# talha-alam/ADAM-Dehaze

Hardware: AMD Instinct MI355X
Metric: images/sec CORUN-Complex fwd+bwd 512x1024 bs=8; PSNR vs CPU ref (higher is better)
Workload: dtype f32; 1 GPU; CORUN-Complex (HighIntensityDehazeModel base 96) train-mode fwd + L1 + bwd + Adam; per_gpu_batch=8, global_batch=8, height=512, width=1024, parallelism=dp1

## Files before the change

adam-dehaze_amd/csrc/bn_act.hip:

```cpp
#include "common.h"

__global__ __launch_bounds__(1024) void bn_finalize_kernel(const float* __restrict__ partials, int nblk, int NcP, int C,
                                                           double count, const float* __restrict__ gamma,
                                                           const float* __restrict__ beta, float eps, float momentum,
                                                           float* running_mean, float* running_var, float* scale,
                                                           float* shift, float* save_mean, float* save_invstd, int64_t* num_batches_tracked) {
    __shared__ double red[2][32][33];
    int c;
    double S, Q, mean, var;
    if (!bn_column_sums<4>(partials, nblk, NcP, C, red, c, S, Q)) return;
    bn_mean_var(S, Q, count, mean, var);
    bn_fold_channel(c, mean, var, count, gamma, beta, eps, momentum, running_mean, running_var, scale, shift, save_mean,
                    save_invstd, num_batches_tracked);
}

extern "C" int adh_bn_finalize(void* stream, const float* partials, int nblk, int NcP, int C, double count,
                               const float* gamma, const float* beta, float eps, float momentum, float* running_mean,
                               float* running_var, float* scale, float* shift, float* save_mean, float* save_invstd,
                               int64_t* num_batches_tracked) {
    if (!partials || !scale || !shift || nblk < 1 || C < 1 || NcP < C || count <= 0) return ADH_E_ARG;
    hipLaunchKernelGGL(bn_finalize_kernel, dim3(adh_ceil_div(C, 32)), dim3(1024), 0, (hipStream_t)stream, partials, nblk,
                       NcP, C, count, gamma, beta, eps, momentum, running_mean, running_var, scale, shift, save_mean,
                       save_invstd, num_batches_tracked);
    return adh_check_launch();
}

__global__ __launch_bounds__(1024) void bn_partial_sums_kernel(const float* __restrict__ partials, int nblk, int pitch, int C,
                                                               double count, double* __restrict__ sums) {
    __shared__ double red[2][32][33];
    int c;
    double S, Q;
    if (bn_column_sums<2>(partials, nblk, pitch, C, red, c, S, Q)) {
        sums[c] = S;
        sums[C + c] = Q;
    }
    if (blockIdx.x == 0 && threadIdx.x == 0) sums[2 * C] = count;
}

extern "C" int adh_bn_partial_sums(void* stream, const float* partials, int nblk, int pitch, int C, double count, double* sums) {
    if (!partials || !sums || nblk < 1 || C < 1 || pitch < C || count <= 0) return ADH_E_ARG;
    hipLaunchKernelGGL(bn_partial_sums_kernel, dim3(adh_ceil_div(C, 32)), dim3(1024), 0, (hipStream_t)stream, partials, nblk,
                       pitch, C, count, sums);
    return adh_check_launch();
}

__global__ void bn_finalize_sums_kernel(const double* __restrict__ sums, int C, const float* __restrict__ gamma,
                                        const float* __restrict__ beta, float eps, float momentum, float* running_mean,
                                        float* running_var, float* scale, float* shift, float* save_mean, float* save_invstd,
                                        int64_t* num_batches_tracked) {
    const int c = blockIdx.x * blockDim.x + threadIdx.x;
    if (c >= C) return;
    const double count = sums[2 * C];
    double mean, var;
    bn_mean_var(sums[c], sums[C + c], count, mean, var);
    bn_fold_channel(c, mean, var, count, gamma, beta, eps, momentum, running_mean, running_var, scale, shift, save_mean,
                    save_invstd, num_batches_tracked);
}

extern "C" int adh_bn_finalize_sums(void* stream, const double* sums, int C, const float* gamma, const float* beta, float eps,
                                    float momentum, float* running_mean, float* running_var, float* scale, float* shift,
                                    float* save_mean, float* save_invstd, int64_t* num_batches_tracked) {
    if (!sums || !scale || !shift || C < 1) return ADH_E_ARG;
    hipLaunchKernelGGL(bn_finalize_sums_kernel, dim3(adh_ceil_div(C, 128)), dim3(128), 0, (hipStream_t)stream, sums, C, gamma,
                       beta, eps, momentum, running_mean, running_var, scale, shift, save_mean, save_invstd, num_batches_tracked);
    return adh_check_launch();
}

__global__ void bn_bwd_finalize_sums_kernel(const double* __restrict__ local_sums, const double* __restrict__ global_sums, int C,
                                            const float* gamma, const float* invstd, float* dgamma, float* dbeta,
                                            int accumulate, float* coef) {
    const int c = blockIdx.x * blockDim.x + threadIdx.x;
    if (c >= C) return;
    const double count = global_sums[2 * C];
    bn_bwd_coef_channel(c, C, local_sums[c], local_sums[C + c], global_sums[c], global_sums[C + c], count, gamma, invstd, dgamma,
// ... 124 lines not shown
        const f32x4 mu = *reinterpret_cast<const f32x4*>(mean + c);
        const f32x4 is = *reinterpret_cast<const f32x4*>(invstd + c);
        f32x4 msc = {0.f, 0.f, 0.f, 0.f}, msh = msc;
        if (mask_ss) {
            msc = *reinterpret_cast<const f32x4*>(mask_ss + c);
            msh = *reinterpret_cast<const f32x4*>(mask_ss + C + c);
        }
        const int64_t p0 = (int64_t)blockIdx.x * BNB_PPB;
        const int64_t p1 = p0 + BNB_PPB < P ? p0 + BNB_PPB : P;
        for (int64_t p = p0 + prow; p < p1; p += BNB_UNROLL * R) {
            f32x4 g[BNB_UNROLL], o[BNB_UNROLL], yy[BNB_UNROLL];
            int mb[BNB_UNROLL];
#pragma unroll
            for (int u = 0; u < BNB_UNROLL; ++u) {
                const int64_t q = p + u * R < p1 ? p + u * R : p;
                g[u] = __builtin_nontemporal_load(reinterpret_cast<const f32x4*>(g_out + q * g_cs + c));
                if (mask_bits) mb[u] = mask_bits[(q * (C / 4) + (c >> 2)) >> 1] >> (4 * ((c >> 2) & 1));
                else if (act == ADH_ACT_RELU && !mask_ss) o[u] = __builtin_nontemporal_load(reinterpret_cast<const f32x4*>(out + q * out_cs + c));
                yy[u] = __builtin_nontemporal_load(reinterpret_cast<const f32x4*>(y + q * y_cs + c));
            }
#pragma unroll
            for (int u = 0; u < BNB_UNROLL; ++u) {
                if (p + u * R < p1) {
                    const f32x4 gg = bn_masked_grad(g[u], act, mask_bits != nullptr, mb[u], mask_ss != nullptr, yy[u], msc, msh, o[u]);
                    sg += gg;
                    sgx += gg * ((yy[u] - mu) * is);
                }
            }
        }
    }
    bn_block_fold(red, sg, sgx, CQ, R, c, C, partials);
  }
}

extern "C" int adh_bn_bwd_reduce(void* stream, const float* g_out, int g_cs, const float* out, int out_cs, int act,
                                 const float* y, int y_cs, const float* mean, const float* invstd, float* partials,
                                 int64_t P, int C, const float* mask_ss, const uint8_t* mask_bits) {
    if (!g_out || !y || !mean || !invstd || !partials || P < 1 || C < 4 || (C & 3) || C > 4096) return ADH_E_ARG;
    if (act == ADH_ACT_RELU && !out && !mask_ss && !mask_bits) return ADH_E_ARG;
    if (mask_bits && (((C / 4) & 1) || act != ADH_ACT_RELU)) return ADH_E_ARG;
    if (!adh_act_host_valid(act) || (act > ADH_ACT_RELU && !mask_ss)) return ADH_E_ARG;
    hipLaunchKernelGGL(bn_bwd_reduce_kernel, dim3(adh_bn_bwd_num_blocks(P, C)), dim3(256), 0, (hipStream_t)stream, g_out,
                       g_cs, out, out_cs, act, y, y_cs, mean, invstd, partials, P, C, mask_ss, mask_bits);
    return adh_check_launch();
}

__global__ __launch_bounds__(1024) void bn_bwd_finalize_kernel(const float* __restrict__ partials, int nblk, int pitch, int C,
                                                               double count, const float* gamma, const float* invstd,
                                                               float* dgamma, float* dbeta, int accumulate, float* coef,
                                                               int centered) {
    __shared__ double red[2][32][33];
    int c;
    double S, Q;
    if (!bn_column_sums<4>(partials, nblk, pitch, C, red, c, S, Q)) return;
    if (centered) Q *= (double)invstd[c];
    bn_bwd_coef_channel(c, C, S, Q, S, Q, count, gamma, invstd, dgamma, dbeta, accumulate, coef);
}

extern "C" int adh_bn_bwd_finalize(void* stream, const float* partials, int nblk, int C, double count,
                                   const float* gamma, const float* invstd, float* dgamma, float* dbeta, int accumulate,
                                   float* coef) {
    if (!partials || !invstd || !coef || nblk < 1 || C < 1 || count <= 0) return ADH_E_ARG;
    hipLaunchKernelGGL(bn_bwd_finalize_kernel, dim3(adh_ceil_div(C, 32)), dim3(1024), 0, (hipStream_t)stream, partials,
                       nblk, C, C, count, gamma, invstd, dgamma, dbeta, accumulate, coef, 0);
    return adh_check_launch();
}

extern "C" int adh_bn_bwd_finalize_centered(void* stream, const float* partials, int nblk, int pitch, int C, double count,
                                            const float* gamma, const float* invstd, float* dgamma, float* dbeta,
                                            int accumulate, float* coef) {
    if (!partials || !invstd || !coef || nblk < 1 || C < 1 || pitch < C || count <= 0) return ADH_E_ARG;
    hipLaunchKernelGGL(bn_bwd_finalize_kernel, dim3(adh_ceil_div(C, 32)), dim3(1024), 0, (hipStream_t)stream, partials,
                       nblk, pitch, C, count, gamma, invstd, dgamma, dbeta, accumulate, coef, 1);
    return adh_check_launch();
}

__global__ __launch_bounds__(256) void bn_bwd_apply_kernel(const float* __restrict__ g_out, int g_cs,
                                                           const float* __restrict__ out, int out_cs, int act,
                                                           const float* __restrict__ y, int y_cs,
                                                           const float* __restrict__ mean,
                                                           const float* __restrict__ invstd,
                                                           const float* __restrict__ coef, int training,
                                                           float* __restrict__ g_y, int gy_cs, float* __restrict__ g_res,
                                                           int gres_cs, int64_t P, int C, const float* __restrict__ mask_ss,
                                                           const uint8_t* __restrict__ mask_bits) {
    const int CQ = C / 4;
    int64_t p, pstep;
    int c;
    adh_stream_decode(CQ, p, pstep, c);
    const f32x4 k0 = *reinterpret_cast<const f32x4*>(coef + c);
    f32x4 mg = {0.f, 0.f, 0.f, 0.f}, kx = mg, mu = mg, msc = mg, msh = mg;
    if (mask_ss) {
        msc = *reinterpret_cast<const f32x4*>(mask_ss + c);
        msh = *reinterpret_cast<const f32x4*>(mask_ss + C + c);
    }
    if (training) {
        mg = *reinterpret_cast<const f32x4*>(coef + C + c);
        const f32x4 mgx = *reinterpret_cast<const f32x4*>(coef + 2 * C + c);
        mu = *reinterpret_cast<const f32x4*>(mean + c);
        kx = *reinterpret_cast<const f32x4*>(invstd + c) * mgx;
    }
    for (; p < P; p += EW_UNROLL * pstep) {
        f32x4 g[EW_UNROLL], o[EW_UNROLL], yy[EW_UNROLL];
        int mb[EW_UNROLL];
#pragma unroll
        for (int u = 0; u < EW_UNROLL; ++u) {
            const int64_t q = p + u * pstep < P ? p + u * pstep : p;
            g[u] = __builtin_nontemporal_load(reinterpret_cast<const f32x4*>(g_out + q * g_cs + c));
            if (mask_bits) mb[u] = mask_bits[(q * CQ + (c >> 2)) >> 1] >> (4 * ((c >> 2) & 1));
            else if (act == ADH_ACT_RELU && !mask_ss) o[u] = __builtin_nontemporal_load(reinterpret_cast<const f32x4*>(out + q * out_cs + c));
            if (training || mask_ss) yy[u] = __builtin_nontemporal_load(reinterpret_cast<const f32x4*>(y + q * y_cs + c));
        }
#pragma unroll
        for (int u = 0; u < EW_UNROLL; ++u) {
            const int64_t q = p + u * pstep;
            if (q < P) {
                f32x4 gg = g[u];
                if (mask_bits) {
#pragma unroll
                    for (int j = 0; j < 4; ++j) gg[j] = ((mb[u] >> j) & 1) ? gg[j] : 0.f;
                } else if (act == ADH_ACT_RELU) {
#pragma unroll
                    for (int j = 0; j < 4; ++j) {
                        const float ov = mask_ss ? fmaf(yy[u][j], msc[j], msh[j]) : o[u][j];
                        gg[j] = ov > 0.f ? gg[j] : 0.f;
// ... 31 lines not shown
```

adam-dehaze_amd/csrc/bn_stream.h:

```cpp
#pragma once

__host__ __device__ static inline bool adh_act_valid(int act) {
    return act == ADH_ACT_NONE || act == ADH_ACT_RELU || act == ADH_ACT_RELU6 || act == ADH_ACT_HARDSWISH ||
           act == ADH_ACT_HARDSIGMOID;
}
static inline bool adh_act_host_valid(int act) { return adh_act_valid(act); }
__device__ __forceinline__ float adh_act_fwd(int act, float z) {
    switch (act) {
        case ADH_ACT_RELU: return fmaxf(z, 0.f);
        case ADH_ACT_RELU6: return fminf(fmaxf(z, 0.f), 6.f);
        case ADH_ACT_HARDSWISH: return z * fminf(fmaxf(z + 3.f, 0.f), 6.f) / 6.f;
        case ADH_ACT_HARDSIGMOID: return fminf(fmaxf(z + 3.f, 0.f), 6.f) / 6.f;
        default: return z;
    }
}
__device__ __forceinline__ float adh_act_bwd(int act, float z, float g) {
    switch (act) {
        case ADH_ACT_RELU: return z > 0.f ? g : 0.f;
        case ADH_ACT_RELU6: return (z > 0.f && z < 6.f) ? g : 0.f;
        case ADH_ACT_HARDSWISH: return z <= -3.f ? 0.f : (z < 3.f ? g * (z / 3.f + 0.5f) : g);
        case ADH_ACT_HARDSIGMOID: return (z > -3.f && z < 3.f) ? g / 6.f : 0.f;
        default: return g;
    }
}
// ... 7 lines not shown
    int64_t blocks = (want + mult - 1) / mult * mult;
    if (blocks < mult) blocks = mult;
    return (int)blocks;
}
__device__ __forceinline__ void adh_stream_decode(int CQ, int64_t& p, int64_t& pstep, int& c) {
    const int64_t t = blockIdx.x * (int64_t)256 + threadIdx.x;
    pstep = (int64_t)gridDim.x * 256 / CQ;
    p = t / CQ;
    c = (int)(t - p * CQ) * 4;
}

__device__ __forceinline__ f32x4 bn_masked_grad(f32x4 gg, int act, bool bits, const int& mb, bool ss, const f32x4& yy,
                                                const f32x4& msc, const f32x4& msh, const f32x4& o) {
    if (bits) {
#pragma unroll
        for (int j = 0; j < 4; ++j) gg[j] = ((mb >> j) & 1) ? gg[j] : 0.f;
    } else if (act == ADH_ACT_RELU) {
#pragma unroll
        for (int j = 0; j < 4; ++j) {
            const float ov = ss ? fmaf(yy[j], msc[j], msh[j]) : o[j];
            gg[j] = ov > 0.f ? gg[j] : 0.f;
        }
    } else if (act != ADH_ACT_NONE) {
#pragma unroll
        for (int j = 0; j < 4; ++j) gg[j] = adh_act_bwd(act, fmaf(yy[j], msc[j], msh[j]), gg[j]);
    }
    return gg;
}

__device__ __forceinline__ void bn_group_decode(int C, int cbase, int& CQ, int& R, int& prow, int& c) {
    CQ = (C - cbase < 1024 ? C - cbase : 1024) / 4;
    R = 256 / CQ;
    const int cq = threadIdx.x % CQ;
    prow = threadIdx.x / CQ;
    c = cbase + cq * 4;
}
__device__ __forceinline__ void bn_block_fold(f32x4 (&red)[2][256], const f32x4& a, const f32x4& b, int CQ, int R, int c, int C,
                                              float* partials) {
    red[0][threadIdx.x] = a;
    red[1][threadIdx.x] = b;
    __syncthreads();
    if (threadIdx.x < CQ) {
        f32x4 sa = {0.f, 0.f, 0.f, 0.f}, sb = {0.f, 0.f, 0.f, 0.f};
        for (int r = 0; r < R; ++r) {
            sa += red[0][r * CQ + threadIdx.x];
            sb += red[1][r * CQ + threadIdx.x];
        }
        *reinterpret_cast<f32x4*>(partials + ((size_t)blockIdx.x * 2 + 0) * C + c) = sa;
        *reinterpret_cast<f32x4*>(partials + ((size_t)blockIdx.x * 2 + 1) * C + c) = sb;
    }
    __syncthreads();
}

template <int CHAINS>
__device__ __forceinline__ bool bn_column_sums(const float* __restrict__ partials, int nblk, int pitch, int C,
                                               double (&red)[2][32][33], int& c, double& S, double& Q) {
    static_assert(CHAINS == 2 || CHAINS == 4, "two or four chains");
    const int cx = threadIdx.x & 31, ry = threadIdx.x >> 5;
    c = blockIdx.x * 32 + cx;
    double s[CHAINS] = {}, q[CHAINS] = {};
    if (c < C) {
        int b = ry;
        for (; b + 32 * (CHAINS - 1) < nblk; b += 32 * CHAINS) {
#pragma unroll
            for (int k = 0; k < CHAINS; ++k) {
                s[k] += (double)partials[((size_t)(b + 32 * k) * 2 + 0) * pitch + c];
                q[k] += (double)partials[((size_t)(b + 32 * k) * 2 + 1) * pitch + c];
            }
        }
        for (; b < nblk; b += 32) {
            s[0] += (double)partials[((size_t)b * 2 + 0) * pitch + c];
            q[0] += (double)partials[((size_t)b * 2 + 1) * pitch + c];
        }
    }
    if constexpr (CHAINS == 4) {
        red[0][ry][cx] = (s[0] + s[1]) + (s[2] + s[3]);
        red[1][ry][cx] = (q[0] + q[1]) + (q[2] + q[3]);
    } else {
        red[0][ry][cx] = s[0] + s[1];
        red[1][ry][cx] = q[0] + q[1];
    }
    __syncthreads();
    if (ry != 0 || c >= C) return false;
    S = 0.0;
    Q = 0.0;
    for (int r = 0; r < 32; ++r) {
        S += red[0][r][cx];
        Q += red[1][r][cx];
    }
    return true;
}

__device__ __forceinline__ void bn_mean_var(double S, double Q, double count, double& mean, double& var) {
    mean = S / count;
    var = Q / count - mean * mean;
    if (var < 0.0) var = 0.0;
}

__device__ __forceinline__ void bn_fold_channel(int c, double mean, double var, double count, const float* __restrict__ gamma,
                                                const float* __restrict__ beta, float eps, float momentum, float* running_mean,
                                                float* running_var, float* scale, float* shift, float* save_mean,
                                                float* save_invstd, int64_t* num_batches_tracked) {
    const double invstd = 1.0 / sqrt(var + (double)eps);
    const float gm = gamma ? gamma[c] : 1.f;
    const float bt = beta ? beta[c] : 0.f;
    scale[c] = (float)(gm * invstd);
    shift[c] = (float)(bt - mean * gm * invstd);
    if (save_mean) save_mean[c] = (float)mean;
    if (save_invstd) save_invstd[c] = (float)invstd;
    if (running_mean) running_mean[c] = (1.f - momentum) * running_mean[c] + momentum * (float)mean;
    if (running_var) {
        const double unbiased = count > 1.0 ? var * count / (count - 1.0) : var;
        running_var[c] = (1.f - momentum) * running_var[c] + momentum * (float)unbiased;
    }
    if (num_batches_tracked && c == 0) *num_batches_tracked += 1;
}

__device__ __forceinline__ void bn_bwd_coef_channel(int c, int C, double dS, double dQ, double mS, double mQ, double count,
                                                    const float* gamma, const float* invstd, float* dgamma, float* dbeta,
                                                    int accumulate, float* coef) {
    if (dgamma) dgamma[c] = accumulate ? dgamma[c] + (float)dQ : (float)dQ;
    if (dbeta) dbeta[c] = accumulate ? dbeta[c] + (float)dS : (float)dS;
    coef[0 * C + c] = (gamma ? gamma[c] : 1.f) * invstd[c];
    coef[1 * C + c] = (float)(mS / count);
    coef[2 * C + c] = (float)(mQ / count);
}
```

adam-dehaze_amd/csrc/cbam.hip:

```cpp
#include "common.h"

#ifndef POOL_PPB
#define POOL_PPB 512
#endif
#ifndef CBAM_SCALE_MAXBLK
#define CBAM_SCALE_MAXBLK 65536
#endif
#ifndef CBAM_ROW_MAXBLK
#define CBAM_ROW_MAXBLK 2048
#endif

extern "C" int adh_cbam_pool_num_blocks(int HW) { return adh_ceil_div(HW, POOL_PPB); }

__global__ __launch_bounds__(256) void cbam_pool_partial_kernel(const float* __restrict__ x, int x_cs, int HW, int C,
                                                                float* __restrict__ partial,
                                                                int32_t* __restrict__ partial_idx, int nblk) {
    __shared__ f32x4 rs[256];
    __shared__ f32x4 rm[256];
    __shared__ int ri[256][4];
    const int n = blockIdx.y, blk = blockIdx.x;
    const int CQ = C / 4;
    const int R = 256 / CQ;
    const int cq = threadIdx.x % CQ, prow = threadIdx.x / CQ;
    const int c = cq * 4;
// ... 268 lines not shown
        }
    }
}

extern "C" int adh_cbam_apply(void* stream, const float* x, int x_cs, const float* ca, const float* smap,
                              const float* wsp, int N, int H, int W, int C, float* sa, float* out, int out_cs) {
    if (!x || !ca || !smap || !wsp || !sa || !out || N < 1 || H < 1 || W < 1 || C < 4 || (C & 3) || (x_cs & 3) || (out_cs & 3) ||
        N > 65535)
        return ADH_E_ARG;
    hipStream_t s = (hipStream_t)stream;
    hipLaunchKernelGGL(cbam_sa_kernel, dim3(adh_ceil_div(W, SA_TW), adh_ceil_div(H, SA_TH), N), dim3(256), 0, s, smap, wsp, H, W,
                       sa);
    hipLaunchKernelGGL(cbam_scale_kernel, dim3(adh_stream_blocks((int64_t)H * W, C / 4, 8, CBAM_SCALE_MAXBLK), N), dim3(256), 0, s,
                       x, x_cs, ca, sa, (int64_t)H * W, C / 4, out, out_cs);
    return adh_check_launch();
}

__global__ __launch_bounds__(256) void cbam_bwd_a_kernel(const float* __restrict__ g, int g_cs,
                                                         const float* __restrict__ x, int x_cs,
                                                         const float* __restrict__ ca, const float* __restrict__ sa,
                                                         int HW, int C, float* __restrict__ gsa_pre) {
    const int n = blockIdx.y;
    const int sub = threadIdx.x & 7;
    const int CQ = C / 4;
    const float* xn = x + (size_t)n * HW * x_cs;
    const float* gn = g + (size_t)n * HW * g_cs;
    const float* can = ca + (size_t)n * C;
    for (int p = blockIdx.x * 32 + (threadIdx.x >> 3); p < HW; p += gridDim.x * 32) {
        float s = 0.f;
        for (int q = sub; q < CQ; q += 8) {
            const f32x4 v = __builtin_nontemporal_load(reinterpret_cast<const f32x4*>(xn + (size_t)p * x_cs + q * 4)) *
                            *reinterpret_cast<const f32x4*>(can + q * 4) *
                            __builtin_nontemporal_load(reinterpret_cast<const f32x4*>(gn + (size_t)p * g_cs + q * 4));
            s += (v[0] + v[1]) + (v[2] + v[3]);
        }
#pragma unroll
        for (int o = 4; o > 0; o >>= 1) s += __shfl_xor(s, o, 64);
        if (sub == 0) {
            const float a = sa[(size_t)n * HW + p];
            gsa_pre[(size_t)n * HW + p] = s * a * (1.f - a);
        }
    }
}

extern "C" int adh_cbam_bwd_a(void* stream, const float* g, int g_cs, const float* x, int x_cs, const float* ca,
                              const float* sa, int N, int HW, int C, float* gsa_pre) {
    if (!g || !x || !ca || !sa || !gsa_pre || N < 1 || HW < 1 || C < 4 || (C & 3)) return ADH_E_ARG;
    const int blocks = adh_min_i(adh_ceil_div(HW, 32), CBAM_ROW_MAXBLK);
    hipLaunchKernelGGL(cbam_bwd_a_kernel, dim3(blocks, N), dim3(256), 0, (hipStream_t)stream, g, g_cs, x, x_cs, ca, sa, HW,
                       C, gsa_pre);
    return adh_check_launch();
}

extern "C" int adh_cbam_bwd_b_num_blocks(int N, int H, int W) { return adh_ceil_div((int64_t)N * H * W, 256); }

__global__ __launch_bounds__(256) void cbam_bwd_b_kernel(const float* __restrict__ gsa_pre,
                                                         const float* __restrict__ smap, const float* __restrict__ wsp,
                                                         int N, int H, int W, float* __restrict__ gsmap,
                                                         float* __restrict__ dwsp_partial) {
    __shared__ float s_w[98];
    __shared__ float s_acc[4][98];
    if (threadIdx.x < 98) s_w[threadIdx.x] = wsp[threadIdx.x];
    __syncthreads();
    const int64_t total = (int64_t)N * H * W;
    const int64_t idx = (int64_t)blockIdx.x * 256 + threadIdx.x;
    const bool valid = idx < total;
    int n = 0, y = 0, xx = 0;
    if (valid) {
        xx = (int)(idx % W);
        const int64_t r = idx / W;
        y = (int)(r % H);
        n = (int)(r / H);
    }
    const float* gp = gsa_pre + (size_t)n * H * W;
    const float* sm = smap + (size_t)n * H * W * 2;
    const float gs_here = valid ? gp[(size_t)y * W + xx] : 0.f;
    float g0 = 0.f, g1 = 0.f;
    const int wave = threadIdx.x >> 6, lane = threadIdx.x & 63;
    for (int ky = 0; ky < 7; ++ky) {
        for (int kx = 0; kx < 7; ++kx) {
            const int oy = y - ky + 3, ox = xx - kx + 3;
            if (valid && oy >= 0 && oy < H && ox >= 0 && ox < W) {
                const float go = gp[(size_t)oy * W + ox];
                g0 += go * s_w[ky * 7 + kx];
                g1 += go * s_w[49 + ky * 7 + kx];
            }
            const int iy = y + ky - 3, ix = xx + kx - 3;
            float a0 = 0.f, a1 = 0.f;
            if (valid && iy >= 0 && iy < H && ix >= 0 && ix < W) {
                const float* q = sm + ((size_t)iy * W + ix) * 2;
                a0 = q[0] * gs_here;
                a1 = q[1] * gs_here;
            }
            a0 = wave_sum(a0);
            a1 = wave_sum(a1);
            if (lane == 0) {
                s_acc[wave][ky * 7 + kx] = a0;
                s_acc[wave][49 + ky * 7 + kx] = a1;
            }
        }
    }
    if (valid) {
        gsmap[idx * 2 + 0] = g0;
        gsmap[idx * 2 + 1] = g1;
    }
    __syncthreads();
    if (threadIdx.x < 98)
        dwsp_partial[(size_t)blockIdx.x * 98 + threadIdx.x] =
            (s_acc[0][threadIdx.x] + s_acc[1][threadIdx.x]) + (s_acc[2][threadIdx.x] + s_acc[3][threadIdx.x]);
}

__global__ __launch_bounds__(256) void cbam_dwsp_final_kernel(const float* __restrict__ partial, int nblk, float* dwsp,
                                                              int accumulate) {
    __shared__ double red[256];
    const int o = blockIdx.x;
    double s = 0.0;
    for (int b = threadIdx.x; b < nblk; b += 256) s += (double)partial[(size_t)b * 98 + o];
    red[threadIdx.x] = s;
    __syncthreads();
    for (int st = 128; st > 0; st >>= 1) {
        if (threadIdx.x < st) red[threadIdx.x] += red[threadIdx.x + st];
        __syncthreads();
    }
    if (threadIdx.x == 0) dwsp[o] = accumulate ? dwsp[o] + (float)red[0] : (float)red[0];
}

extern "C" int adh_cbam_bwd_b(void* stream, const float* gsa_pre, const float* smap, const float* wsp, int N, int H,
                              int W, float* gsmap, float* dwsp_partial, int nblk, float* dwsp, int accumulate) {
    if (!gsa_pre || !smap || !wsp || !gsmap || !dwsp_partial || !dwsp) return ADH_E_ARG;
    if (nblk != adh_cbam_bwd_b_num_blocks(N, H, W)) return ADH_E_ARG;
    hipStream_t s = (hipStream_t)stream;
    hipLaunchKernelGGL(cbam_bwd_b_kernel, dim3(nblk), dim3(256), 0, s, gsa_pre, smap, wsp, N, H, W, gsmap, dwsp_partial);
    hipLaunchKernelGGL(cbam_dwsp_final_kernel, dim3(98), dim3(256), 0, s, dwsp_partial, nblk, dwsp, accumulate);
    return adh_check_launch();
}

__device__ __forceinline__ f32x4 cbam_gx1(const f32x4 g, float sa, float gmean_over_c, float gmax, int cidx, int c) {
    f32x4 r = g * sa + gmean_over_c;
#pragma unroll
    for (int j = 0; j < 4; ++j)
        if (c + j == cidx) r[j] += gmax;
    return r;
}

__global__ __launch_bounds__(256) void cbam_bwd_c_kernel(const float* __restrict__ g, int g_cs,
                                                         const float* __restrict__ x, int x_cs,
                                                         const float* __restrict__ sa, const float* __restrict__ gsmap,
                                                         const int32_t* __restrict__ cidx, int HW, int C,
                                                         float* __restrict__ gca_partial, int nblk) {
    __shared__ f32x4 rs[256];
    const int n = blockIdx.y, blk = blockIdx.x;
    const int CQ = C / 4;
    const int R = 256 / CQ;
    const int cq = threadIdx.x % CQ, prow = threadIdx.x / CQ;
    const int c = cq * 4;
    const float invC = 1.0f / (float)C;
    f32x4 s = {0.f, 0.f, 0.f, 0.f};
    if (prow < R) {
        const float* xn = x + (size_t)n * HW * x_cs;
        const float* gn = g + (size_t)n * HW * g_cs;
        const int p0 = blk * POOL_PPB;
        const int p1 = adh_min_i(p0 + POOL_PPB, HW);
        for (int p = p0 + prow; p < p1; p += 4 * R) {
            f32x4 gv[4], xv[4];
            float sv[4], gm[4], gx[4];
            int ci[4];
#pragma unroll
            for (int u = 0; u < 4; ++u) {
                const int q = p + u * R < p1 ? p + u * R : p;
                const size_t pp = (size_t)n * HW + q;
                gv[u] = __builtin_nontemporal_load(reinterpret_cast<const f32x4*>(gn + (size_t)q * g_cs + c));
                xv[u] = __builtin_nontemporal_load(reinterpret_cast<const f32x4*>(xn + (size_t)q * x_cs + c));
                sv[u] = sa[pp];
                gm[u] = gsmap[pp * 2 + 0];
                gx[u] = gsmap[pp * 2 + 1];
                ci[u] = cidx[pp];
            }
#pragma unroll
            for (int u = 0; u < 4; ++u)
                if (p + u * R < p1) s += cbam_gx1(gv[u], sv[u], gm[u] * invC, gx[u], ci[u], c) * xv[u];
        }
    }
    rs[threadIdx.x] = s;
    __syncthreads();
    if (threadIdx.x < CQ) {
        f32x4 S = {0.f, 0.f, 0.f, 0.f};
// ... 172 lines not shown
```

adam-dehaze_amd/csrc/common.h:

```cpp
#pragma once
#include <hip/hip_runtime.h>
#include <stdint.h>
#include "../../include/adam_dehaze_hip.h"

typedef float f32x4 __attribute__((ext_vector_type(4)));
typedef float f32x16 __attribute__((ext_vector_type(16)));

#define ADH_WAVE 64

#define ADH_ADAM_CHUNK 16384

#define ADH_DYN_LDS(T, name) extern __shared__ __attribute__((aligned(16))) T name[]

static inline int adh_check_launch() {
    hipError_t e = hipGetLastError();
    return e == hipSuccess ? ADH_OK : ADH_E_LAUNCH;
}

__host__ __device__ static inline int adh_min_i(int a, int b) { return a < b ? a : b; }
__host__ __device__ static inline int adh_max_i(int a, int b) { return a > b ? a : b; }
static inline int adh_ceil_div(int64_t a, int64_t b) { return (int)((a + b - 1) / b); }
static inline int adh_round_up(int a, int b) { return (a + b - 1) / b * b; }

__host__ __device__ static inline int adh_tap_min(int d0, int step, int k) {
// ... 6 lines not shown
}

struct ConvGeom {
    int dmin_y, dmin_x;
    int halo_h, halo_w;
    int npx, npxp;
    int tiles_x, tiles_y;
    int KC, KQ_log2;
    int KQtot;
    int TH;
    int xp;
};

#include "wave.h"
__device__ __forceinline__ float sigmoidf_(float v) { return 1.0f / (1.0f + __expf(-v)); }

__device__ __forceinline__ float adh_opaque(float v) {
    asm volatile("" : "+s"(v));
    return v;
}
__device__ __forceinline__ f32x4 adh_pksub(const f32x4& a, const f32x4& b, float m1) { return m1 * b + a; }

template <int TN>
__device__ __forceinline__ void adh_mfma_operand_fence(float (&V)[4], float (&M)[TN][4]) {
    if constexpr (TN == 1)
        asm volatile("s_nop 1" : "+v"(V[0]), "+v"(V[1]), "+v"(V[2]), "+v"(V[3]), "+v"(M[0][0]), "+v"(M[0][1]), "+v"(M[0][2]), "+v"(M[0][3]));
    if constexpr (TN == 2)
        asm volatile("s_nop 1" : "+v"(V[0]), "+v"(V[1]), "+v"(V[2]), "+v"(V[3]), "+v"(M[0][0]), "+v"(M[0][1]), "+v"(M[0][2]), "+v"(M[0][3]),
                     "+v"(M[1][0]), "+v"(M[1][1]), "+v"(M[1][2]), "+v"(M[1][3]));
    if constexpr (TN == 3)
        asm volatile("s_nop 1" : "+v"(V[0]), "+v"(V[1]), "+v"(V[2]), "+v"(V[3]), "+v"(M[0][0]), "+v"(M[0][1]), "+v"(M[0][2]), "+v"(M[0][3]),
                     "+v"(M[1][0]), "+v"(M[1][1]), "+v"(M[1][2]), "+v"(M[1][3]), "+v"(M[2][0]), "+v"(M[2][1]), "+v"(M[2][2]), "+v"(M[2][3]));
}

__host__ __device__ static inline int64_t adh_wlayout_tap_off(const adh_wlayout& L, int ty, int tx) {
    return (int64_t)L.tap_off0 + ty * L.tap_off_sy + tx * L.tap_off_sx;
}
__host__ __device__ static inline int64_t adh_wlayout_off(const adh_wlayout& L, int ty, int tx, int k, int n) {
    return adh_wlayout_tap_off(L, ty, tx) + (int64_t)k * L.stride_k + (int64_t)n * L.stride_n;
}

static inline int adh_split_grid_blocks(int nsplit, int ngroups) { return ((nsplit + 7) / 8) * ngroups * 8; }
__device__ __forceinline__ void adh_split_grid_decode(int bid, int ngroups, int& group, int& split) {
    const int q = bid >> 3;
    group = q % ngroups;
    split = (q / ngroups) * 8 + (bid & 7);
}

#define G4_A 0.75f
#define G4_B 1.25f

void adh_wgrad_sum_splits(hipStream_t s, float* slab, int nsplit, int64_t n4);

struct adh_wg32_taps {
    int ncls;
    int tap0[4], tap_sy[4], tap_sx[4], rev[4];
};
int adh_wgrad32_class_taps(const adh_conv_desc* d, adh_wg32_taps* tp);

int adh_rows_fwd_num_blocks(const adh_conv_desc* d);
int adh_rows_fwd_launch(void* stream, const adh_conv_desc* d);

#include "bn_stream.h"
```

adam-dehaze_amd/csrc/conv_wgrad.hip:

```cpp
#include "common.h"
#include <cstdlib>

#define WG_TW 32

template <int T, int TN>
__global__ __launch_bounds__(512, 2) void conv_wgrad_kernel(const adh_conv_desc d, const ConvGeom g, float* slab,
                                                            int ntiles, int KP, int nco_groups) {
    extern __shared__ __attribute__((aligned(16))) float smem[];
    constexpr int BN = 32 * TN;
    constexpr int PER = (T * TN + 3) / 4;
    const int XP = g.xp;
    const int buf_floats = g.npx * XP + 32 + g.TH * WG_TW * BN;

    const int tid = threadIdx.x;
    const int lane = tid & 63;
    const int wave = __builtin_amdgcn_readfirstlane(tid >> 6);
    const bool loader = wave >= 4;
    const int l31 = lane & 31;
    const int h = lane >> 5;

    const int ci_tile = blockIdx.x / nco_groups;
    const int co_grp = blockIdx.x - ci_tile * nco_groups;
    const int ci0 = ci_tile * 32;
    const int co0 = co_grp * BN;
// ... 585 lines not shown
    const int nblocks = adh_split_grid_blocks(nsplit, p.a.ngroups);
    hipStream_t s = (hipStream_t)stream;
#define WW_CASE(tn_) \
    if (p.TN == tn_) { \
        (void)hipFuncSetAttribute(reinterpret_cast<const void*>(&conv_wgrad_rows_kernel<3, 3, false, tn_, true>), \
                                  hipFuncAttributeMaxDynamicSharedMemorySize, 160 * 1024); \
        hipLaunchKernelGGL((conv_wgrad_rows_kernel<3, 3, false, tn_, true>), dim3(nblocks), dim3(256), lds, s, *d, p.a, slab); \
        return adh_check_launch(); \
    }
    WW_CASE(3) WW_CASE(2) WW_CASE(1)
#undef WW_CASE
    return ADH_E_UNSUPPORTED;
}

extern "C" int adh_conv_wgrad_groups(const adh_conv_desc* d) {
    if (!d) return ADH_E_ARG;
    WrPlan plan[4];
    const int n = wgrad_rows_plan(d, 1, plan);
    return n && wgrad_rows_instantiated(plan[0]) ? plan[0].a.ngroups : 0;
}

extern "C" int adh_conv_wgrad_slabs(const adh_conv_desc* d, int nsplit) {
    if (!d || nsplit < 1) return ADH_E_ARG;
    return adh_conv_wgrad_groups(d) > 0 ? 4 * nsplit : nsplit;
}

extern "C" int adh_conv_wgrad(void* stream, const adh_conv_desc* d, float* slab, int nsplit) {
    if (!d || !slab || nsplit < 1 || !d->in || !d->out) return ADH_E_ARG;
    if (d->NcP % 32 != 0 || d->NcP < d->Cout) return ADH_E_ARG;
    {
        WrPlan plan[4];
        const int np = wgrad_rows_plan(d, nsplit, plan);
        if (np && wgrad_rows_instantiated(plan[0])) {
            for (int i = 0; i < np; ++i) {
                const int rc = dispatch_wgrad_rows((hipStream_t)stream, d, plan[i], slab);
                if (rc) return rc;
            }
            return ADH_OK;
        }
    }
    const int Ttot = d->KH * d->KW;
    int T;
    if (Ttot == 9 || Ttot == 16 || Ttot == 4 || Ttot == 1) T = Ttot;
    else if (Ttot == 49 || Ttot == 14) T = 7;
    else return ADH_E_UNSUPPORTED;
    const bool packed = (d->dstep_x == 4 && d->Cin == 8 && d->in_sx == 1);
    const int TN = wgrad_pick_tn(d->NcP, T);
    ConvGeom g;
    int rc = wgrad_geometry(d, &g, TN, packed ? 8 : 32);
    if (rc) return rc;
    if ((d->VH - 1) * d->out_sy + d->out_oy >= d->OH || (d->VW - 1) * d->out_sx + d->out_ox >= d->OW) return ADH_E_ARG;
    const int KP = adh_round_up(d->Cin, 32);
    hipStream_t s = (hipStream_t)stream;
#define WG_CASE(t, tn) \
    if (T == t && TN == tn) { launch_wgrad<t, tn>(s, d, g, slab, nsplit, KP); return adh_check_launch(); }
    WG_CASE(9, 4) WG_CASE(9, 3) WG_CASE(9, 2) WG_CASE(9, 1)
    WG_CASE(16, 3) WG_CASE(16, 2) WG_CASE(16, 1)
    WG_CASE(4, 4) WG_CASE(4, 3) WG_CASE(4, 2) WG_CASE(4, 1)
    WG_CASE(7, 4) WG_CASE(7, 3) WG_CASE(7, 2) WG_CASE(7, 1)
    WG_CASE(1, 4) WG_CASE(1, 3) WG_CASE(1, 2) WG_CASE(1, 1)
#undef WG_CASE
    return ADH_E_UNSUPPORTED;
}
```

Measured before the change: 40.41 images/sec.

## Retile BN finalize reductions, tile CBAM spatial backward, add 1x1 small-channel wgrad kernel

BN finalize kernels now reduce 8 channels per block over 128 slices instead of 32x32, giving more blocks and deeper per-channel parallelism for small channel counts. The CBAM spatial-attention backward is rewritten as a persistent tiled kernel that stages gradient and map halos in shared memory, prefetches the next tile in registers, and accumulates the 98 weight gradients in registers. This replaces per-tap wave reductions. A dedicated 1x1 weight-gradient kernel handles tiny Cin/Cout=4 convolutions with vectorized streaming loads. These trade register pressure and extra code paths for fewer redundant loads and reductions.

Result: no change. 40.66 images/sec, median of 6 (+0.6%).

```diff
diff --git a/adam-dehaze_amd/csrc/bn_act.hip b/adam-dehaze_amd/csrc/bn_act.hip
--- a/adam-dehaze_amd/csrc/bn_act.hip
+++ b/adam-dehaze_amd/csrc/bn_act.hip
@@ -8,7 +8,7 @@
     __shared__ double red[2][32][33];
     int c;
     double S, Q, mean, var;
-    if (!bn_column_sums<4>(partials, nblk, NcP, C, red, c, S, Q)) return;
+    if (!bn_column_sums<BN_FIN_CHAINS, BN_FIN_CH>(partials, nblk, NcP, C, red, c, S, Q)) return;
     bn_mean_var(S, Q, count, mean, var);
     bn_fold_channel(c, mean, var, count, gamma, beta, eps, momentum, running_mean, running_var, scale, shift, save_mean,
                     save_invstd, num_batches_tracked);
@@ -19,7 +19,7 @@
                                float* running_var, float* scale, float* shift, float* save_mean, float* save_invstd,
                                int64_t* num_batches_tracked) {
     if (!partials || !scale || !shift || nblk < 1 || C < 1 || NcP < C || count <= 0) return ADH_E_ARG;
-    hipLaunchKernelGGL(bn_finalize_kernel, dim3(adh_ceil_div(C, 32)), dim3(1024), 0, (hipStream_t)stream, partials, nblk,
+    hipLaunchKernelGGL(bn_finalize_kernel, dim3(bn_finalize_blocks(C)), dim3(1024), 0, (hipStream_t)stream, partials, nblk,
                        NcP, C, count, gamma, beta, eps, momentum, running_mean, running_var, scale, shift, save_mean,
                        save_invstd, num_batches_tracked);
     return adh_check_launch();
@@ -250,7 +250,7 @@
     __shared__ double red[2][32][33];
     int c;
     double S, Q;
-    if (!bn_column_sums<4>(partials, nblk, pitch, C, red, c, S, Q)) return;
+    if (!bn_column_sums<BN_FIN_CHAINS, BN_FIN_CH>(partials, nblk, pitch, C, red, c, S, Q)) return;
     if (centered) Q *= (double)invstd[c];
     bn_bwd_coef_channel(c, C, S, Q, S, Q, count, gamma, invstd, dgamma, dbeta, accumulate, coef);
 }
@@ -259,7 +259,7 @@
                                    const float* gamma, const float* invstd, float* dgamma, float* dbeta, int accumulate,
                                    float* coef) {
     if (!partials || !invstd || !coef || nblk < 1 || C < 1 || count <= 0) return ADH_E_ARG;
-    hipLaunchKernelGGL(bn_bwd_finalize_kernel, dim3(adh_ceil_div(C, 32)), dim3(1024), 0, (hipStream_t)stream, partials,
+    hipLaunchKernelGGL(bn_bwd_finalize_kernel, dim3(bn_finalize_blocks(C)), dim3(1024), 0, (hipStream_t)stream, partials,
                        nblk, C, C, count, gamma, invstd, dgamma, dbeta, accumulate, coef, 0);
     return adh_check_launch();
 }
@@ -268,7 +268,7 @@
                                             const float* gamma, const float* invstd, float* dgamma, float* dbeta,
                                             int accumulate, float* coef) {
     if (!partials || !invstd || !coef || nblk < 1 || C < 1 || pitch < C || count <= 0) return ADH_E_ARG;
-    hipLaunchKernelGGL(bn_bwd_finalize_kernel, dim3(adh_ceil_div(C, 32)), dim3(1024), 0, (hipStream_t)stream, partials,
+    hipLaunchKernelGGL(bn_bwd_finalize_kernel, dim3(bn_finalize_blocks(C)), dim3(1024), 0, (hipStream_t)stream, partials,
                        nblk, pitch, C, count, gamma, invstd, dgamma, dbeta, accumulate, coef, 1);
     return adh_check_launch();
 }
diff --git a/adam-dehaze_amd/csrc/bn_stream.h b/adam-dehaze_amd/csrc/bn_stream.h
--- a/adam-dehaze_amd/csrc/bn_stream.h
+++ b/adam-dehaze_amd/csrc/bn_stream.h
@@ -83,44 +83,86 @@
     __syncthreads();
 }
 
-template <int CHAINS>
+#define BN_FIN_CH 8
+#define BN_FIN_CHAINS 4
+template <int CHAINS, int CH = 32>
 __device__ __forceinline__ bool bn_column_sums(const float* __restrict__ partials, int nblk, int pitch, int C,
                                                double (&red)[2][32][33], int& c, double& S, double& Q) {
-    static_assert(CHAINS == 2 || CHAINS == 4, "two or four chains");
-    const int cx = threadIdx.x & 31, ry = threadIdx.x >> 5;
-    c = blockIdx.x * 32 + cx;
+    static_assert(CHAINS == 2 || CHAINS == 4 || CHAINS == 8, "two, four or eight chains");
+    static_assert((CH == 32 && CHAINS <= 4) || CH == 8, "32 channels x 32 slices or 8 channels x 128 slices");
+    constexpr int SL = 1024 / CH;
+    const int cx = threadIdx.x % CH, ry = threadIdx.x / CH;
+    c = blockIdx.x * CH + cx;
     double s[CHAINS] = {}, q[CHAINS] = {};
     if (c < C) {
         int b = ry;
-        for (; b + 32 * (CHAINS - 1) < nblk; b += 32 * CHAINS) {
+        for (; b + SL * (CHAINS - 1) < nblk; b += SL * CHAINS) {
 #pragma unroll
             for (int k = 0; k < CHAINS; ++k) {
-                s[k] += (double)partials[((size_t)(b + 32 * k) * 2 + 0) * pitch + c];
-                q[k] += (double)partials[((size_t)(b + 32 * k) * 2 + 1) * pitch + c];
+                s[k] += (double)partials[((size_t)(b + SL * k) * 2 + 0) * pitch + c];
+                q[k] += (double)partials[((size_t)(b + SL * k) * 2 + 1) * pitch + c];
             }
         }
-        for (; b < nblk; b += 32) {
+        for (; b < nblk; b += SL) {
             s[0] += (double)partials[((size_t)b * 2 + 0) * pitch + c];
             q[0] += (double)partials[((size_t)b * 2 + 1) * pitch + c];
         }
     }
-    if constexpr (CHAINS == 4) {
-        red[0][ry][cx] = (s[0] + s[1]) + (s[2] + s[3]);
-        red[1][ry][cx] = (q[0] + q[1]) + (q[2] + q[3]);
+    double ts, tq;
+    if constexpr (CHAINS == 8) {
+        ts = ((s[0] + s[1]) + (s[2] + s[3])) + ((s[4] + s[5]) + (s[6] + s[7]));
+        tq = ((q[0] + q[1]) + (q[2] + q[3])) + ((q[4] + q[5]) + (q[6] + q[7]));
+    } else if constexpr (CHAINS == 4) {
+        ts = (s[0] + s[1]) + (s[2] + s[3]);
+        tq = (q[0] + q[1]) + (q[2] + q[3]);
     } else {
-        red[0][ry][cx] = s[0] + s[1];
-        red[1][ry][cx] = q[0] + q[1];
-    }
-    __syncthreads();
-    if (ry != 0 || c >= C) return false;
-    S = 0.0;
-    Q = 0.0;
-    for (int r = 0; r < 32; ++r) {
-        S += red[0][r][cx];
-        Q += red[1][r][cx];
-    }
-    return true;
-}
+        ts = s[0] + s[1];
+        tq = q[0] + q[1];
+    }
+    if constexpr (CH == 32) {
+        red[0][ry][cx] = ts;
+        red[1][ry][cx] = tq;
+        __syncthreads();
+        if (ry != 0 || c >= C) return false;
+        S = 0.0;
+        Q = 0.0;
+        for (int r = 0; r < 32; ++r) {
+            S += red[0][r][cx];
+            Q += red[1][r][cx];
+        }
+        return true;
+    } else {
+        double* fs = &red[0][0][0];
+        double* fq = &red[1][0][0];
+        fs[threadIdx.x] = ts;
+        fq[threadIdx.x] = tq;
+        __syncthreads();
+        double gsum = 0.0, gq = 0.0;
+        if (ry < SL / 8) {
+#pragma unroll
+            for (int r = 0; r < 8; ++r) {
+                gsum += fs[(ry * 8 + r) * CH + cx];
+                gq += fq[(ry * 8 + r) * CH + cx];
+            }
+        }
+        __syncthreads();
+        if (ry < SL / 8) {
+            fs[threadIdx.x] = gsum;
+            fq[threadIdx.x] = gq;
+        }
+        __syncthreads();
+        if (ry != 0 || c >= C) return false;
+        S = 0.0;
+        Q = 0.0;
+#pragma unroll
+        for (int r = 0; r < SL / 8; ++r) {
+            S += fs[r * CH + cx];
+            Q += fq[r * CH + cx];
+        }
+        return true;
+    }
+}
+static inline int bn_finalize_blocks(int C) { return (C + BN_FIN_CH - 1) / BN_FIN_CH; }
 
 __device__ __forceinline__ void bn_mean_var(double S, double Q, double count, double& mean, double& var) {
     mean = S / count;
diff --git a/adam-dehaze_amd/csrc/cbam.hip b/adam-dehaze_amd/csrc/cbam.hip
--- a/adam-dehaze_amd/csrc/cbam.hip
+++ b/adam-dehaze_amd/csrc/cbam.hip
@@ -344,62 +344,144 @@
     return adh_check_launch();
 }
 
+#define BB_TW 64
+#define BB_SH 4
+#define BB_TH (4 * BB_SH)
+#define BB_LP (BB_TW + 6)
+#define BB_ELEMS ((BB_TH + 6) * BB_LP)
+#define BB_LD ((BB_ELEMS + 255) / 256)
+#ifndef BB_MAXBLK
+#define BB_MAXBLK 256
+#endif
 extern "C" int adh_cbam_bwd_b_num_blocks(int N, int H, int W) { return adh_ceil_div((int64_t)N * H * W, 256); }
 
 __global__ __launch_bounds__(256) void cbam_bwd_b_kernel(const float* __restrict__ gsa_pre,
                                                          const float* __restrict__ smap, const float* __restrict__ wsp,
                                                          int N, int H, int W, float* __restrict__ gsmap,
-                                                         float* __restrict__ dwsp_partial) {
-    __shared__ float s_w[98];
-    __shared__ float s_acc[4][98];
-    if (threadIdx.x < 98) s_w[threadIdx.x] = wsp[threadIdx.x];
-    __syncthreads();
-    const int64_t total = (int64_t)N * H * W;
-    const int64_t idx = (int64_t)blockIdx.x * 256 + threadIdx.x;
-    const bool valid = idx < total;
-    int n = 0, y = 0, xx = 0;
-    if (valid) {
-        xx = (int)(idx % W);
-        const int64_t r = idx / W;
-        y = (int)(r % H);
-        n = (int)(r / H);
-    }
-    const float* gp = gsa_pre + (size_t)n * H * W;
-    const float* sm = smap + (size_t)n * H * W * 2;
-    const float gs_here = valid ? gp[(size_t)y * W + xx] : 0.f;
-    float g0 = 0.f, g1 = 0.f;
-    const int wave = threadIdx.x >> 6, lane = threadIdx.x & 63;
-    for (int ky = 0; ky < 7; ++ky) {
-        for (int kx = 0; kx < 7; ++kx) {
-            const int oy = y - ky + 3, ox = xx - kx + 3;
-            if (valid && oy >= 0 && oy < H && ox >= 0 && ox < W) {
-                const float go = gp[(size_t)oy * W + ox];
-                g0 += go * s_w[ky * 7 + kx];
-                g1 += go * s_w[49 + ky * 7 + kx];
-            }
-            const int iy = y + ky - 3, ix = xx + kx - 3;
-            float a0 = 0.f, a1 = 0.f;
-            if (valid && iy >= 0 && iy < H && ix >= 0 && ix < W) {
-                const float* q = sm + ((size_t)iy * W + ix) * 2;
-                a0 = q[0] * gs_here;
-                a1 = q[1] * gs_here;
-            }
-            a0 = wave_sum(a0);
-            a1 = wave_sum(a1);
-            if (lane == 0) {
-                s_acc[wave][ky * 7 + kx] = a0;
-                s_acc[wave][49 + ky * 7 + kx] = a1;
-            }
-        }
-    }
-    if (valid) {
-        gsmap[idx * 2 + 0] = g0;
-        gsmap[idx * 2 + 1] = g1;
-    }
-    __syncthreads();
-    if (threadIdx.x < 98)
-        dwsp_partial[(size_t)blockIdx.x * 98 + threadIdx.x] =
-            (s_acc[0][threadIdx.x] + s_acc[1][threadIdx.x]) + (s_acc[2][threadIdx.x] + s_acc[3][threadIdx.x]);
+                                                         float* __restrict__ dwsp_partial, int nblk) {
+    __shared__ float tg[BB_ELEMS];
+    __shared__ float ts0[BB_ELEMS];
+    __shared__ float ts1[BB_ELEMS];
+    __shared__ float s_red[14][257];
+    __shared__ float s_part[98][17];
+    const int tiles_x = (W + BB_TW - 1) / BB_TW, tiles_y = (H + BB_TH - 1) / BB_TH;
+    const int64_t tiles_img = (int64_t)tiles_x * tiles_y, ntiles = tiles_img * N;
+    const int lx = threadIdx.x & 63, ly0 = (threadIdx.x >> 6) * BB_SH;
+    float dw0[49], dw1[49];
+#pragma unroll
+    for (int i = 0; i < 49; ++i) dw0[i] = dw1[i] = 0.f;
+
+    float pg[BB_LD], pa[BB_LD], pb[BB_LD];
+    auto tile_origin = [&](int64_t t, int& n, int& y0, int& x0) {
+        n = (int)(t / tiles_img);
+        const int rem = (int)(t - n * tiles_img);
+        y0 = (rem / tiles_x) * BB_TH;
+        x0 = (rem % tiles_x) * BB_TW;
+    };
+    auto fetch = [&](int64_t t) {
+        int n, y0, x0;
+        tile_origin(t, n, y0, x0);
+#pragma unroll
+        for (int k = 0; k < BB_LD; ++k) {
+            const int i = threadIdx.x + 256 * k;
+            const int r = i / BB_LP, cc = i - r * BB_LP;
+            const int yy = y0 + r - 3, xx = x0 + cc - 3;
+            const bool ok = i < BB_ELEMS && yy >= 0 && yy < H && xx >= 0 && xx < W;
+            const size_t p = ok ? ((size_t)n * H + yy) * W + xx : 0;
+            pg[k] = gsa_pre[p];
+            pa[k] = smap[p * 2];
+            pb[k] = smap[p * 2 + 1];
+            if (!ok) pg[k] = pa[k] = pb[k] = 0.f;
+        }
+    };
+    if ((int64_t)blockIdx.x < ntiles) fetch(blockIdx.x);
+    for (int64_t t = blockIdx.x; t < ntiles; t += gridDim.x) {
+        int n, y0, x0;
+        tile_origin(t, n, y0, x0);
+#pragma unroll
+        for (int k = 0; k < BB_LD; ++k) {
+            const int i = threadIdx.x + 256 * k;
+            if (i < BB_ELEMS) {
+                tg[i] = pg[k];
+                ts0[i] = pa[k];
+                ts1[i] = pb[k];
+            }
+        }
+        __syncthreads();
+        if (t + gridDim.x < ntiles) fetch(t + gridDim.x);
+        float gs[BB_SH], g0[BB_SH], g1[BB_SH];
+#pragma unroll
+        for (int j = 0; j < BB_SH; ++j) {
+            gs[j] = tg[(ly0 + j + 3) * BB_LP + lx + 3];
+            g0[j] = g1[j] = 0.f;
+        }
+#pragma unroll
+        for (int r = BB_SH + 5; r >= 0; --r) {
+            float grow[7], s0[7], s1[7];
+#pragma unroll
+            for (int c = 0; c < 7; ++c) {
+                grow[c] = tg[(ly0 + r) * BB_LP + lx + c];
+                s0[c] = ts0[(ly0 + r) * BB_LP + lx + c];
+                s1[c] = ts1[(ly0 + r) * BB_LP + lx + c];
+            }
+#pragma unroll
+            for (int j = 0; j < BB_SH; ++j) {
+                const int ky = j + 6 - r;
+                if (ky >= 0 && ky < 7) {
+#pragma unroll
+                    for (int kx = 0; kx < 7; ++kx) {
+                        const float go = grow[6 - kx];
+                        g0[j] += go * wsp[ky * 7 + kx];
+                        g1[j] += go * wsp[49 + ky * 7 + kx];
+                    }
+                }
+                const int kv = r - j;
+                if (kv >= 0 && kv < 7) {
+#pragma unroll
+                    for (int kx = 0; kx < 7; ++kx) {
+                        dw0[kv * 7 + kx] += s0[kx] * gs[j];
+                        dw1[kv * 7 + kx] += s1[kx] * gs[j];
+                    }
+                }
+            }
+        }
+        const int x = x0 + lx;
+#pragma unroll
+        for (int j = 0; j < BB_SH; ++j) {
+            const int y = y0 + ly0 + j;
+            if (y < H && x < W) {
+                float* o = gsmap + (((size_t)n * H + y) * W + x) * 2;
+                o[0] = g0[j];
+                o[1] = g1[j];
+            }
+        }
+        __syncthreads();
+    }
+#pragma unroll
+    for (int p = 0; p < 7; ++p) {
+#pragma unroll
+        for (int i = 0; i < 14; ++i) {
+            const int o = p * 14 + i;
+            s_red[i][threadIdx.x] = o < 49 ? dw0[o < 49 ? o : 0] : dw1[o < 49 ? 0 : o - 49];
+        }
+        __syncthreads();
+        if (threadIdx.x < 14 * 16) {
+            const int i = threadIdx.x >> 4, part = threadIdx.x & 15;
+            float s = 0.f;
+#pragma unroll
+            for (int k = 0; k < 16; ++k) s += s_red[i][part * 16 + k];
+            s_part[p * 14 + i][part] = s;
+        }
+        __syncthreads();
+    }
+    if (threadIdx.x < 98) {
+        float s = 0.f;
+#pragma unroll
+        for (int k = 0; k < 16; ++k) s += s_part[threadIdx.x][k];
+        dwsp_partial[(size_t)blockIdx.x * 98 + threadIdx.x] = s;
+        for (int64_t row = (int64_t)gridDim.x + blockIdx.x; row < nblk; row += gridDim.x)
+            dwsp_partial[(size_t)row * 98 + threadIdx.x] = 0.f;
+    }
 }
 
 __global__ __launch_bounds__(256) void cbam_dwsp_final_kernel(const float* __restrict__ partial, int nblk, float* dwsp,
@@ -422,8 +504,10 @@
     if (!gsa_pre || !smap || !wsp || !gsmap || !dwsp_partial || !dwsp) return ADH_E_ARG;
     if (nblk != adh_cbam_bwd_b_num_blocks(N, H, W)) return ADH_E_ARG;
     hipStream_t s = (hipStream_t)stream;
-    hipLaunchKernelGGL(cbam_bwd_b_kernel, dim3(nblk), dim3(256), 0, s, gsa_pre, smap, wsp, N, H, W, gsmap, dwsp_partial);
-    hipLaunchKernelGGL(cbam_dwsp_final_kernel, dim3(98), dim3(256), 0, s, dwsp_partial, nblk, dwsp, accumulate);
+    const int64_t ntiles = (int64_t)N * adh_ceil_div(H, BB_TH) * adh_ceil_div(W, BB_TW);
+    const int grid = (int)(ntiles < adh_min_i(nblk, BB_MAXBLK) ? ntiles : adh_min_i(nblk, BB_MAXBLK));
+    hipLaunchKernelGGL(cbam_bwd_b_kernel, dim3(grid), dim3(256), 0, s, gsa_pre, smap, wsp, N, H, W, gsmap, dwsp_partial, nblk);
+    hipLaunchKernelGGL(cbam_dwsp_final_kernel, dim3(98), dim3(256), 0, s, dwsp_partial, grid, dwsp, accumulate);
     return adh_check_launch();
 }
 
diff --git a/adam-dehaze_amd/csrc/common.h b/adam-dehaze_amd/csrc/common.h
--- a/adam-dehaze_amd/csrc/common.h
+++ b/adam-dehaze_amd/csrc/common.h
@@ -82,6 +82,8 @@
 
 void adh_wgrad_sum_splits(hipStream_t s, float* slab, int nsplit, int64_t n4);
 
+int adh_conv_wgrad_1x1_stream(hipStream_t s, const adh_conv_desc* d, float* slab, int nsplit);
+
 struct adh_wg32_taps {
     int ncls;
     int tap0[4], tap_sy[4], tap_sx[4], rev[4];
diff --git a/adam-dehaze_amd/csrc/conv_wgrad.hip b/adam-dehaze_amd/csrc/conv_wgrad.hip
--- a/adam-dehaze_amd/csrc/conv_wgrad.hip
+++ b/adam-dehaze_amd/csrc/conv_wgrad.hip
@@ -661,6 +661,7 @@
     if ((d->VH - 1) * d->out_sy + d->out_oy >= d->OH || (d->VW - 1) * d->out_sx + d->out_ox >= d->OW) return ADH_E_ARG;
     const int KP = adh_round_up(d->Cin, 32);
     hipStream_t s = (hipStream_t)stream;
+    if (adh_conv_wgrad_1x1_stream(s, d, slab, nsplit)) return adh_check_launch();
 #define WG_CASE(t, tn) \
     if (T == t && TN == tn) { launch_wgrad<t, tn>(s, d, g, slab, nsplit, KP); return adh_check_launch(); }
     WG_CASE(9, 4) WG_CASE(9, 3) WG_CASE(9, 2) WG_CASE(9, 1)
diff --git a/adam-dehaze_amd/csrc/conv_wgrad_1x1.hip b/adam-dehaze_amd/csrc/conv_wgrad_1x1.hip
--- /dev/null
+++ b/adam-dehaze_amd/csrc/conv_wgrad_1x1.hip
@@ -0,0 +1,91 @@
+#include "common.h"
+
+#define W1_UNROLL 8
+
+__global__ __launch_bounds__(256) void conv_wgrad_1x1_kernel(const adh_conv_desc d, float* __restrict__ slab, int64_t total,
+                                                             int dense) {
+    __shared__ float red[16][257];
+    __shared__ float res[16][4];
+    const int CQ = d.Cin / 4;
+    const int R = 256 / CQ;
+    const int q = threadIdx.x % CQ, lane = threadIdx.x / CQ;
+    const int nsplit = gridDim.x;
+    const int64_t per = (total + nsplit - 1) / nsplit;
+    const int64_t m0 = (int64_t)blockIdx.x * per;
+    const int64_t m1 = m0 + per < total ? m0 + per : total;
+    const int64_t vhw = (int64_t)d.VH * d.VW;
+
+    float acc[4][4];
+#pragma unroll
+    for (int i = 0; i < 4; ++i)
+#pragma unroll
+        for (int j = 0; j < 4; ++j) acc[i][j] = 0.f;
+
+    if (lane < R) {
+        for (int64_t mb = m0 + lane; mb < m1; mb += (int64_t)R * W1_UNROLL) {
+            f32x4 xv[W1_UNROLL], gv[W1_UNROLL];
+#pragma unroll
+            for (int u = 0; u < W1_UNROLL; ++u) {
+                const int64_t m = mb + (int64_t)u * R;
+                const f32x4 zero = {0.f, 0.f, 0.f, 0.f};
+                xv[u] = zero;
+                gv[u] = zero;
+                if (m < m1) {
+                    if (dense) {
+                        xv[u] = __builtin_nontemporal_load(reinterpret_cast<const f32x4*>(d.in + (size_t)m * d.in_cstride + q * 4));
+                        gv[u] = __builtin_nontemporal_load(reinterpret_cast<const f32x4*>(d.out + (size_t)m * d.out_cstride));
+                    } else {
+                        const int n = (int)(m / vhw);
+                        const int rem = (int)(m - n * vhw);
+                        const int vy = rem / d.VW, vx = rem - vy * d.VW;
+                        const int iy = vy * d.in_sy + d.dy0, ix = vx * d.in_sx + d.dx0;
+                        const int oy = vy * d.out_sy + d.out_oy, ox = vx * d.out_sx + d.out_ox;
+                        if (iy >= 0 && iy < d.IH && ix >= 0 && ix < d.IW) {
+                            xv[u] = *reinterpret_cast<const f32x4*>(d.in + (((size_t)n * d.IH + iy) * d.IW + ix) * d.in_cstride + q * 4);
+                            gv[u] = *reinterpret_cast<const f32x4*>(d.out + (((size_t)n * d.OH + oy) * d.OW + ox) * d.out_cstride);
+                        }
+                    }
+                }
+            }
+#pragma unroll
+            for (int u = 0; u < W1_UNROLL; ++u)
+#pragma unroll
+                for (int i = 0; i < 4; ++i)
+#pragma unroll
+                    for (int j = 0; j < 4; ++j) acc[i][j] += xv[u][i] * gv[u][j];
+        }
+    }
+#pragma unroll
+    for (int i = 0; i < 4; ++i)
+#pragma unroll
+        for (int j = 0; j < 4; ++j) red[i * 4 + j][threadIdx.x] = acc[i][j];
+    __syncthreads();
+    if (threadIdx.x < CQ * 16) {
+        const int qq = threadIdx.x / 16, e = threadIdx.x % 16;
+        float s = 0.f;
+        for (int r = 0; r < R; ++r) s += red[e][r * CQ + qq];
+        res[qq * 4 + e / 4][e % 4] = s;
+    }
+    __syncthreads();
+    {
+        const int ci = threadIdx.x >> 3, cq = threadIdx.x & 7;
+        f32x4 v = {0.f, 0.f, 0.f, 0.f};
+        if (cq == 0 && ci < d.Cin) {
+#pragma unroll
+            for (int j = 0; j < 4; ++j) v[j] = res[ci][j];
+        }
+        *reinterpret_cast<f32x4*>(slab + (size_t)blockIdx.x * 1024 + threadIdx.x * 4) = v;
+    }
+}
+
+int adh_conv_wgrad_1x1_stream(hipStream_t s, const adh_conv_desc* d, float* slab, int nsplit) {
+    if (d->KH != 1 || d->KW != 1 || d->Cin < 4 || d->Cin > 16 || (d->Cin & 3) || d->Cout != 4 || d->NcP != 32) return 0;
+    if ((d->in_cstride & 3) || (d->out_cstride & 3) || d->in_cstride < d->Cin || d->out_cstride < d->Cout) return 0;
+    if (d->N < 1 || d->VH < 1 || d->VW < 1) return 0;
+    const int64_t total = (int64_t)d->N * d->VH * d->VW;
+    if (total >= ((int64_t)1 << 31) || (int64_t)d->VH * d->VW >= ((int64_t)1 << 31)) return 0;
+    const int dense = d->in_sy == 1 && d->in_sx == 1 && d->dy0 == 0 && d->dx0 == 0 && d->out_sy == 1 && d->out_sx == 1 &&
+                      d->out_oy == 0 && d->out_ox == 0 && d->VH == d->IH && d->VW == d->IW && d->VH == d->OH && d->VW == d->OW;
+    hipLaunchKernelGGL(conv_wgrad_1x1_kernel, dim3(nsplit), dim3(256), 0, s, *d, slab, total, dense);
+    return 1;
+}
```
